# tongdaxu/VQ-VAE-from-Gaussian-VAE

Hardware: AMD Instinct MI355X
Metric: images/sec encode+quantize+decode, 256x256, codebook 2^16 (higher is better)
Workload: dtype f32

## Files before the change

vq-vae-from-gaussian-vae_amd/csrc/gq_unet_aux.h:

```cpp
#pragma once
#include "gq_common.h"
#include "gq_stats.h"

namespace gqhip {

typedef unsigned u32x4_t __attribute__((ext_vector_type(4)));

__device__ __forceinline__ float silu_f32(float x) {
  const float d = 1.0f + __expf(-x);
  const float r = __builtin_amdgcn_rcpf(d);
  const float q = x * r;
  const float q1 = __builtin_fmaf(__builtin_fmaf(-d, q, x), r, q);
  return d > 1e37f ? q : q1;
}

template <int SILU, typename VEC>
__device__ __forceinline__ VEC gn_act(VEC v, VEC a, VEC sh) {
  v = v * a + sh;
  if (SILU) {
#pragma unroll
    for (int e = 0; e < (int)(sizeof(VEC) / sizeof(float)); ++e) v[e] = silu_f32(v[e]);
  }
  return v;
}
__global__ __launch_bounds__(256) void gn_stats_nhwc_kernel(const float *__restrict__ x,
                                                            const float *__restrict__ pre_bias,
                                                            int64_t *__restrict__ stats, int C, long HW, int cpg,
                                                            int slabs) {
  __shared__ int64_t red[kStatWords * 64];
  const int groups = C / cpg, quads = C / 4, lanes = 256 / quads;
  const long b = blockIdx.x / slabs;
  const int slab = blockIdx.x % slabs;
  const long per = (HW + slabs - 1) / slabs;
  const long lo = slab * per, hi = lo + per < HW ? lo + per : HW;
  const int q = threadIdx.x % quads, pl = threadIdx.x / quads;
// ... 246 lines not shown
          d[i][j] = reinterpret_cast<const f32x4 *>(x)[((wt.b * H + sy) * W + sx) * C4 + wt.q];
      }
    f32x4 w[4][4];
#pragma unroll
    for (int j = 0; j < 4; ++j) {
      w[0][j] = d[0][j] - d[2][j];
      w[1][j] = d[1][j] + d[2][j];
      w[2][j] = d[2][j] - d[1][j];
      w[3][j] = d[1][j] - d[3][j];
    }
    f32x4 *v = reinterpret_cast<f32x4 *>(V);
#pragma unroll
    for (int i = 0; i < 4; ++i) {
      v[((long)(4 * i + 0) * tiles + wt.tile) * C4 + wt.q] = w[i][0] - w[i][2];
      v[((long)(4 * i + 1) * tiles + wt.tile) * C4 + wt.q] = w[i][1] + w[i][2];
      v[((long)(4 * i + 2) * tiles + wt.tile) * C4 + wt.q] = w[i][2] - w[i][1];
      v[((long)(4 * i + 3) * tiles + wt.tile) * C4 + wt.q] = w[i][1] - w[i][3];
    }
  }
}
template <int F16X3>
__global__ __launch_bounds__(256) void wino_in_nhwc_kernel(const float *__restrict__ x, void *__restrict__ V, int H, int W,
                                                           int C4, long tiles, long total, float scale) {
  if constexpr (F16X3 == 0) wino_in_items_f32(x, static_cast<float *>(V), H, W, C4, tiles, total);
  else wino_in_items<F16X3, uint32_t>(x, V, H, W, C4, tiles, total, scale);
}
template <int F16X3>
__global__ __launch_bounds__(256) void wino_in_nhwc_wide_kernel(const float *__restrict__ x, void *__restrict__ V, int H, int W,
                                                                int C4, long tiles, long total, float scale) {
  if constexpr (F16X3 == 0) wino_in_items_f32(x, static_cast<float *>(V), H, W, C4, tiles, total);
  else wino_in_items<F16X3, uint64_t>(x, V, H, W, C4, tiles, total, scale);
}

template <int SILU, int F16X3, typename OFF>
__device__ __forceinline__ void wino_in_gn_items(const float *__restrict__ x, const float *__restrict__ gamma,
                                                 const float *__restrict__ beta, const float *__restrict__ pre_bias,
                                                 const int64_t *__restrict__ stats, void *__restrict__ V, int H, int W, int C4,
                                                 int cpg, double eps, long tiles, long total, float scale) {
  typedef WinoVRow<F16X3, f32x4> VR;
  const int groups = 4 * C4 / cpg;
  const OFF px = (OFF)C4 * sizeof(f32x4), row = (OFF)W * px;
  const OFF part = (OFF)C4 * VR::VB;
  const uint64_t plane = (uint64_t)tiles * VR::PARTS * part;
  const char *xb = reinterpret_cast<const char *>(x);
  for (OFF t = (OFF)blockIdx.x * 256 + threadIdx.x; t < (OFF)total; t += (OFF)gridDim.x * 256) {
    const WinoTile<OFF> wt = wino_tile<2>(t, C4, H, W);
    char *vk = wino_plane0(static_cast<char *>(V));
    const int g = (4 * wt.q) / cpg;
    const GnGroup gg = gn_group(stats + kStatWords * ((long)wt.b * groups + g), (double)cpg * (double)H * (double)W, eps);
    f32x4 a, sh;
#pragma unroll
    for (int k = 0; k < 4; ++k) {
      const GnAffine f = gn_channel(gg, gamma, beta, pre_bias, 4 * wt.q + k);
      a[k] = f.a;
      sh[k] = f.sh;
    }
    const OFF xq = wt.b * ((OFF)H * row) + (OFF)wt.q * sizeof(f32x4);
    OFF ro[4], co[4];
    float rin[4], cin[4];
    wino_taps<4>(2 * wt.th - 1, H, row, xq, ro, rin);
    wino_taps<4>(2 * wt.tw - 1, W, px, (OFF)0, co, cin);
    f32x4 d[4][4];
#pragma unroll
    for (int i = 0; i < 4; ++i)
#pragma unroll
      for (int j = 0; j < 4; ++j) {
        d[i][j] = *reinterpret_cast<const f32x4 *>(xb + (OFF)(ro[i] + co[j]));
      }
#pragma unroll
    for (int i = 0; i < 4; ++i)
#pragma unroll
      for (int j = 0; j < 4; ++j) {
        const float inb = rin[i] * cin[j];
        d[i][j] = gn_act<SILU>(d[i][j], a, sh) * inb;
      }
    f32x4 w[4][4];
#pragma unroll
    for (int j = 0; j < 4; ++j) {
      w[0][j] = d[0][j] - d[2][j];
      w[1][j] = d[1][j] + d[2][j];
      w[2][j] = d[2][j] - d[1][j];
      w[3][j] = d[1][j] - d[3][j];
    }
    const OFF at = wt.tile * (VR::PARTS * part) + (OFF)wt.q * VR::VB;
#pragma unroll
    for (int i = 0; i < 4; ++i) {
      wino_store_v<F16X3>(vk, at, part, w[i][0] - w[i][2], scale);
      vk += plane;
      wino_store_v<F16X3>(vk, at, part, w[i][1] + w[i][2], scale);
      vk += plane;
      wino_store_v<F16X3>(vk, at, part, w[i][2] - w[i][1], scale);
      vk += plane;
      wino_store_v<F16X3>(vk, at, part, w[i][1] - w[i][3], scale);
      vk += plane;
    }
  }
}
#define GQ_WINO_GN_ARGS                                                                                                        \
  const float *__restrict__ x, const float *__restrict__ gamma, const float *__restrict__ beta,                               \
      const float *__restrict__ pre_bias, const int64_t *__restrict__ stats, void *__restrict__ V, int H, int W, int CV, int cpg, \
      double eps, long tiles, long total, float scale
template <int SILU, int F16X3>
__global__ __launch_bounds__(256) __attribute__((amdgpu_waves_per_eu(3, 4))) void wino_in_gn_nhwc_kernel(GQ_WINO_GN_ARGS) {
  wino_in_gn_items<SILU, F16X3, uint32_t>(x, gamma, beta, pre_bias, stats, V, H, W, CV, cpg, eps, tiles, total, scale);
}
template <int SILU, int F16X3>
__global__ __launch_bounds__(256) void wino_in_gn_nhwc_wide_kernel(GQ_WINO_GN_ARGS) {
  wino_in_gn_items<SILU, F16X3, uint64_t>(x, gamma, beta, pre_bias, stats, V, H, W, CV, cpg, eps, tiles, total, scale);
}

template <int F16X3, typename OFF>
__device__ __forceinline__ void wino4_in_items(const float *__restrict__ x, void *__restrict__ V, int H, int W, int C4, long tiles,
                                               long total, float scale) {
  typedef WinoVRow<F16X3, f32x4> VR;
  const OFF px = (OFF)C4 * sizeof(f32x4), row = (OFF)W * px;
  const OFF part = (OFF)C4 * VR::VB;
  const uint64_t plane = (uint64_t)tiles * VR::PARTS * part;
  const char *xb = reinterpret_cast<const char *>(x);
  for (OFF t = (OFF)blockIdx.x * 256 + threadIdx.x; t < (OFF)total; t += (OFF)gridDim.x * 256) {
    const WinoTile<OFF> wt = wino_tile<4>(t, C4, H, W);
    char *vk = wino_plane0(static_cast<char *>(V));
    const OFF xq = wt.b * ((OFF)H * row) + (OFF)wt.q * sizeof(f32x4);
    OFF ro[6], co[6];
    bool rin[6], cin[6];
    wino_taps<6>(4 * wt.th - 1, H, row, xq, ro, rin);
    wino_taps<6>(4 * wt.tw - 1, W, px, (OFF)0, co, cin);
    f32x4 w[6][6];
#pragma unroll
    for (int j = 0; j < 6; ++j) {
      f32x4 col[6], o[6];
#pragma unroll
      for (int i = 0; i < 6; ++i) {
        col[i] = f32x4{0.f, 0.f, 0.f, 0.f};
        if (rin[i] && cin[j]) col[i] = *reinterpret_cast<const f32x4 *>(xb + (OFF)(ro[i] + co[j]));
      }
      wino4_bt(col, o);
#pragma unroll
      for (int i = 0; i < 6; ++i) w[i][j] = o[i];
    }
    const OFF at = wt.tile * (VR::PARTS * part) + (OFF)wt.q * VR::VB;
#pragma unroll
    for (int i = 0; i < 6; ++i) {
// ... 582 lines not shown
```

vq-vae-from-gaussian-vae_amd/csrc/gq_wino_range.h:

```cpp
#pragma once
#include <stdint.h>

#include <initializer_list>

namespace gqhip {

inline bool wino_product_le(uint64_t a, uint64_t b, uint64_t limit) { return a == 0 || b <= limit / a; }

inline bool wino_offsets_fit_u32(int64_t B, int64_t H, int64_t W, int64_t C, int64_t tile, int64_t plane_bytes_per_channel) {
  if (B < 0 || H < 1 || W < 1 || C < 1 || tile < 1 || plane_bytes_per_channel < 1) return false;
  const uint64_t limit = 1ull << 32;
  uint64_t tensor = 4, plane = (uint64_t)plane_bytes_per_channel;
  for (uint64_t f : {(uint64_t)B, (uint64_t)H, (uint64_t)W, (uint64_t)C}) {
    if (!wino_product_le(tensor, f, limit)) return false;
    tensor *= f;
  }
  for (uint64_t f : {(uint64_t)B, (uint64_t)(H / tile), (uint64_t)(W / tile), (uint64_t)C}) {
    if (!wino_product_le(plane, f, limit)) return false;
    plane *= f;
  }
  return true;
}

}
```

vq-vae-from-gaussian-vae_amd/csrc/gqhip_unet.hip:

```cpp
#include "gqhip.h"

#include <hip/hip_ext.h>
#include <hip/hip_runtime.h>

#include <cstdlib>
#include <initializer_list>
#include <cstring>

#include "gqhip_internal.h"
#include "gq_unet_aux.h"
#include "gq_wino_range.h"
#include "gq_wino_gemm.h"
#include "gq_conv3.h"
#include "gq_conv_f32.h"
#include "gq_attn.h"
#include "gq_attn_bwd.h"

using namespace gqhip;

namespace {
thread_local int g_stats_prezeroed = 0;
inline hipError_t stats_zero(void *p, size_t bytes, hipStream_t st) {
  return g_stats_prezeroed ? hipSuccess : hipMemsetAsync(p, 0, bytes, st);
}

constexpr int kGo = -1;

dim3 grid1d(long total, long cap) {
  const long blocks = (total + 255) / 256;
  return dim3((unsigned)(blocks > cap ? cap : blocks));
}

int nhwc_slabs(int64_t C, int64_t HW) {
  const int lanes = (int)(256 / (C / 4));
  int slabs = (int)((HW + (int64_t)lanes * 16 - 1) / ((int64_t)lanes * 16));
  if (slabs > 1024) slabs = 1024;
  return slabs < 1 ? 1 : slabs;
}

int gn_check(int64_t B, int64_t C, int64_t HW, int64_t groups, bool ptrs_ok, bool nhwc) {
  if (B < 0 || C < 1 || HW < 1 || groups < 1 || C % groups != 0) return GQHIP_ERR_INVALID_ARG;
  if (B == 0) return GQHIP_OK;
  if (!ptrs_ok) return GQHIP_ERR_INVALID_ARG;
  if (nhwc && ((C / groups) % 4 != 0 || 256 % (C / 4) != 0 || groups > 64)) return GQHIP_ERR_INVALID_ARG;
  return kGo;
}

bool wino_shape_ok(int64_t B, int64_t H, int64_t W, int64_t C, int64_t tile) {
  return (tile == 2 || tile == 4) && B >= 0 && H >= tile && W >= tile && H % tile == 0 && W % tile == 0 && C >= 4 && C % 4 == 0;
}
bool wino_u32(int64_t B, int64_t H, int64_t W, int64_t C, int64_t tile, int64_t plane_bytes_per_channel) {
  const char *knob = getenv("GQHIP_WINO_WIDE");
  return !(knob && !strcmp(knob, "1")) && wino_offsets_fit_u32(B, H, W, C, tile, plane_bytes_per_channel);
}

bool one_of(int64_t v, std::initializer_list<int64_t> values) {
  for (int64_t w : values)
    if (v == w) return true;
  return false;
}
}

extern "C" {

int gqhip_stats_prezeroed(int on) {
  g_stats_prezeroed = on != 0;
  return GQHIP_OK;
}

int gn_silu_f32(const float *x, const float *gamma, const float *beta, const float *pre_bias_or_null, float *y,
                int64_t B, int64_t C, int64_t HW, int64_t groups, double eps, int apply_silu, int layout,
                int64_t *stats_ws, void *stream) {
  const bool nhwc = layout == GQHIP_LAYOUT_NHWC;
  if (int rc = gn_check(B, C, HW, groups, x && gamma && beta && y && stats_ws, nhwc); rc != kGo) return rc;
  hipStream_t st = static_cast<hipStream_t>(stream);
  const int64_t bg = B * groups, cpg = C / groups, chunk = cpg * HW;
  if (nhwc) {
    if (stats_zero(stats_ws, sizeof(int64_t) * kStatWords * bg, st) != hipSuccess) return check_launch();
    const int slabs = nhwc_slabs(C, HW);
    hipLaunchKernelGGL(gn_stats_nhwc_kernel, dim3((unsigned)(B * slabs)), dim3(256), 0, st, x, pre_bias_or_null,
                       stats_ws, (int)C, (long)HW, (int)cpg, slabs);
    int rc = check_launch();
    if (rc != GQHIP_OK) return rc;
    return launch(apply_silu ? gn_apply_nhwc_kernel<1> : gn_apply_nhwc_kernel<0>, dim3((unsigned)(B * slabs)), dim3(256), 0, st, x,
                  gamma, beta, y, stats_ws, pre_bias_or_null, (int)C, (long)HW, (int)cpg, eps, slabs);
  }
// ... 111 lines not shown
  wp.nnb = (int)(Cout / cols);
  wp.mtiles = tiles / rows; wp.ntile_total = P * wp.mtiles; wp.tiles_per_xcd = (wp.ntile_total + 7) / 8;
  const long blocks = 8 * wp.tiles_per_xcd * wp.nnb;
  if (blocks > 0x7fffffffL) return GQHIP_ERR_INVALID_ARG;
  hipStream_t st = static_cast<hipStream_t>(stream);
  switch (tiling) {
    case WinoGemmTiling::k128x256: hipLaunchKernelGGL(wino_gemm_f16x2_k64_kernel<1>, dim3((unsigned)blocks), dim3(256), 0, st, wp); break;
    case WinoGemmTiling::k256x256: hipLaunchKernelGGL(wino_gemm_f16x2_k64_kernel<2>, dim3((unsigned)blocks), dim3(512), 0, st, wp); break;
    case WinoGemmTiling::k256x128: hipLaunchKernelGGL(wino_gemm_f16x2_kernel, dim3((unsigned)blocks), dim3(256), 0, st, wp); break;
  }
  return check_launch();
}

int gn_stats_f32(const float *x, const float *pre_bias_or_null, int64_t B, int64_t C, int64_t HW, int64_t groups,
                 int64_t *stats_out, void *stream) {
  if (int rc = gn_check(B, C, HW, groups, x && stats_out, true); rc != kGo) return rc;
  const int64_t cpg = C / groups;
  hipStream_t st = static_cast<hipStream_t>(stream);
  if (stats_zero(stats_out, sizeof(int64_t) * kStatWords * B * groups, st) != hipSuccess) return check_launch();
  const int slabs = nhwc_slabs(C, HW);
  return launch(gn_stats_nhwc_kernel, dim3((unsigned)(B * slabs)), dim3(256), 0, st, x, pre_bias_or_null, stats_out,
                (int)C, (long)HW, (int)cpg, slabs);
}

static int wino_in_gn_impl(int tile, int f16, const float *x, const float *gamma, const float *beta,
                           const float *pre_bias_or_null, const int64_t *stats, void *V, int64_t B, int64_t H, int64_t W,
                           int64_t C, int64_t groups, double eps, int apply_silu, float scale, void *stream) {
  if (!wino_shape_ok(B, H, W, C, tile) || groups < 1 || C % groups != 0 || (C / groups) % 4 != 0 || !(scale > 0.f))
    return GQHIP_ERR_INVALID_ARG;
  if (B == 0) return GQHIP_OK;
  if (!x || !gamma || !beta || !stats || !V) return GQHIP_ERR_INVALID_ARG;
  const int vw = (tile == 4 && f16 != 0) ? 2 : 4;
  const long tiles = (long)(B * (H / tile) * (W / tile)), total = tiles * (C / vw);
  const dim3 grid = grid1d(total, 32768);
  hipStream_t st = static_cast<hipStream_t>(stream);
  const bool u32 = wino_u32(B, H, W, C, tile, f16 == 1 ? 6 : 4);
#define GQ_WGN(K, ...)                                                                                                       \
  hipLaunchKernelGGL((u32 ? K##_kernel<__VA_ARGS__> : K##_wide_kernel<__VA_ARGS__>), grid, dim3(256), 0, st, x, gamma, beta, \
                     pre_bias_or_null, stats, V, (int)H, (int)W, (int)(C / vw), (int)(C / groups), eps, tiles, total, scale)
  if (tile == 4) {
    if (apply_silu) {
      if (f16 == 2) GQ_WGN(wino4_in_gn_nhwc, 1, 2, 2); else if (f16 == 1) GQ_WGN(wino4_in_gn_nhwc, 1, 1, 2);
      else GQ_WGN(wino4_in_gn_nhwc, 1, 0, 4);
    } else {
      if (f16 == 2) GQ_WGN(wino4_in_gn_nhwc, 0, 2, 2); else if (f16 == 1) GQ_WGN(wino4_in_gn_nhwc, 0, 1, 2);
      else GQ_WGN(wino4_in_gn_nhwc, 0, 0, 4);
    }
  } else {
    if (apply_silu) {
      if (f16 == 2) GQ_WGN(wino_in_gn_nhwc, 1, 2); else if (f16 == 1) GQ_WGN(wino_in_gn_nhwc, 1, 1);
      else GQ_WGN(wino_in_gn_nhwc, 1, 0);
    } else {
      if (f16 == 2) GQ_WGN(wino_in_gn_nhwc, 0, 2); else if (f16 == 1) GQ_WGN(wino_in_gn_nhwc, 0, 1);
      else GQ_WGN(wino_in_gn_nhwc, 0, 0);
    }
  }
#undef GQ_WGN
  return check_launch();
}

int wino_in_gn_nhwc_f32(const float *x, const float *gamma, const float *beta, const float *pre_bias_or_null,
                        const int64_t *stats, float *V, int64_t B, int64_t H, int64_t W, int64_t C, int64_t groups,
                        double eps, int apply_silu, void *stream) {
  return wino_in_gn_impl(2, 0, x, gamma, beta, pre_bias_or_null, stats, V, B, H, W, C, groups, eps, apply_silu, 1.0f, stream);
}

int wino4_in_gn_nhwc_f32(const float *x, const float *gamma, const float *beta, const float *pre_bias_or_null,
                         const int64_t *stats, float *V, int64_t B, int64_t H, int64_t W, int64_t C, int64_t groups,
                         double eps, int apply_silu, void *stream) {
// ... 457 lines not shown
```

vq-vae-from-gaussian-vae_amd/csrc/gq_conv3.h:

```cpp
#pragma once
#include <type_traits>

#include "gq_common.h"
#include "gq_epilogue.h"
#include "gq_stats.h"
#include "gq_wino_gemm.h"

namespace gqhip {

constexpr int kC3TH = 8, kC3TW = 32;
constexpr int kC3PH = kC3TH + 2, kC3PW = kC3TW + 2;
constexpr int kC3Pix = kC3PH * kC3PW;
constexpr int kC3RS = 48;
constexpr int kC3Plane = kC3PH * kC3RS * 32;
constexpr int kC3Buf = 2 * kC3Plane;
constexpr int kC3Pieces = kC3Pix * 4;
constexpr int kC3Loads = (kC3Pieces + 255) / 256;

__device__ __forceinline__ int conv3_lds_off(int R, int x, int half) {
  return (R * kC3RS + x) * 32 + 16 * (half ^ ((x >> 3) & 1));
}

struct Conv3Params {
  const _Float16 *Xs;
// ... 75 lines not shown
    double *mine = part + (wn * 64 + lane) * 4;
    if (wm == 0) {
      if (p.res) epi_store<3, true>(acc, stage, lane, p.y, p.res, o, slice, 4 * cout, p.mscale, pb, st);
      else epi_store<2, true>(acc, stage, lane, p.y, nullptr, o, slice, 4 * cout, p.mscale, pb, st);
      mine[0] = st.v0; mine[1] = st.s; mine[2] = st.ss; mine[3] = (double)st.n;
    }
    __syncthreads();
    if (wm == 1) {
      st.v0 = mine[0]; st.s = mine[1]; st.ss = mine[2]; st.n = (int)mine[3];
      if (p.res) epi_store<3, true>(acc, stage, lane, p.y, p.res, o, slice, 4 * cout, p.mscale, pb, st);
      else epi_store<2, true>(acc, stage, lane, p.y, nullptr, o, slice, 4 * cout, p.mscale, pb, st);
      stat_partial_flush(red + kStatWords * (n / p.cpg), st);
    }
  }
  __syncthreads();
  const int gpb = 128 / p.cpg, groups = cout / p.cpg;
  if (tid < kStatWords * gpb) stat_flush_word(p.stats + kStatWords * (t.b * groups + t.nb * gpb) + tid, red[tid]);
}

#define GQ_C3_ZERO_ACC(acc)                                                                                         \
  _Pragma("unroll") for (int rr = 0; rr < 4; ++rr) _Pragma("unroll") for (int j = 0; j < 2; ++j) acc[rr][j] =       \
      f32x16{0.f, 0.f, 0.f, 0.f, 0.f, 0.f, 0.f, 0.f, 0.f, 0.f, 0.f, 0.f, 0.f, 0.f, 0.f, 0.f}

struct Conv3GnParams {
  Conv3Params c;
  const float *x;
  const float *gamma, *beta, *pre_bias;
  const int64_t *stats_in;
  int cin, cpg_in;
  double eps;
  float scale;
};

#ifdef GQHIP_CLOCK_STAMPS
__device__ unsigned long long g_c3_stamps[4 * 8192];
#endif
template <int SILU, int COUT>
__global__ __launch_bounds__(256, 2) void conv3x3_gn_f16x3_kernel(const Conv3GnParams pp) {
  typedef _Float16 f16x4 __attribute__((ext_vector_type(4)));
  const Conv3Params &p = pp.c;
  __shared__ __attribute__((aligned(16))) unsigned char sA[2 * kC3Buf];
  __shared__ int64_t red[kStatWords * 32];
  __shared__ __attribute__((aligned(16))) float sAff[2][512];
  const int tid = threadIdx.x, lane = tid & 63, wave = __builtin_amdgcn_readfirstlane(tid >> 6);
  const int c = lane & 31, h = lane >> 5, wm = wave >> 1, wn = wave & 1;
#ifdef GQHIP_CLOCK_STAMPS
  const unsigned long long st_r0 = __builtin_amdgcn_s_memrealtime();
#endif
  Conv3Tile t;
  if (!conv3_tile(p, t)) return;
  const int H = p.H, W = p.W, cin = pp.cin;
  red[tid] = 0;
  {
    const int groups = cin / pp.cpg_in;
    const double n = (double)pp.cpg_in * (double)H * (double)W;
    for (int ch = tid; ch < cin; ch += 256) {
      const GnAffine f = gn_channel(gn_group(pp.stats_in + kStatWords * (t.b * groups + ch / pp.cpg_in), n, pp.eps), pp.gamma, pp.beta, pp.pre_bias, ch);
      sAff[0][ch] = f.a;
      sAff[1][ch] = f.sh;
    }
  }
  const int w = tid & 3, qs = tid >> 2;
  int goff[kC3Loads];
  unsigned inb = 0;
#pragma unroll
  for (int i = 0; i < kC3Loads; ++i) {
    int q = qs + 64 * i;
    q = q < kC3Pix ? q : kC3Pix - 1;
    const int R = q / kC3PW, px = q % kC3PW;
    const int gy = t.y0 - 1 + R, gx = t.x0 - 1 + px;
    const bool in = gy >= 0 && gy < H && gx >= 0 && gx < W;
    const int cy = clamp_index(gy, H), cx = clamp_index(gx, W);
    goff[i] = (cy * W + cx) * cin + 4 * w;
    inb |= (unsigned)(in ? 1 : 0) << i;
  }
  const float *xb = pp.x + t.b * (long)H * W * cin;
  f32x4 st[3];
  auto issue = [&](int i, int chunk) { st[i % 3] = *reinterpret_cast<const f32x4 *>(xb + goff[i] + chunk * 16); };
  auto convert = [&](int i, int chunk, int buf) {
    const int q = qs + 64 * i;
    if (q >= kC3Pix) return;
    const f32x4 a4 = *reinterpret_cast<const f32x4 *>(&sAff[0][chunk * 16 + 4 * w]);
    const f32x4 sh4 = *reinterpret_cast<const f32x4 *>(&sAff[1][chunk * 16 + 4 * w]);
    const f32x4 v = gn_act<SILU>(st[i % 3], a4, sh4) * (((inb >> i) & 1) ? pp.scale : 0.f);
    f16x4 hi, lo;
#pragma unroll
    for (int e = 0; e < 4; ++e) {
      hi[e] = (_Float16)v[e];
      lo[e] = (_Float16)(v[e] - (float)hi[e]);
    }
    const int off = buf * kC3Buf + conv3_lds_off(q / kC3PW, q % kC3PW, w >> 1) + 8 * (w & 1);
    *reinterpret_cast<f16x4 *>(&sA[off]) = hi;
    *reinterpret_cast<f16x4 *>(&sA[off + kC3Plane]) = lo;
  };

  f32x16 acc[4][2];
  GQ_C3_ZERO_ACC(acc);
  int aoff[3];
#pragma unroll
  for (int dx = 0; dx < 3; ++dx) aoff[dx] = conv3_lds_off(4 * wm, c + dx, h);
  const unsigned char *wbase = reinterpret_cast<const unsigned char *>(p.Wf) + (4 * t.nb + 2 * wn) * 128 * 16;
  const int wl = lane * 16;
  const long wstep = (long)p.nnb * (512 * 16);
  f16x8 bs[3][4];
  auto load_b = [&](int ks, f16x8 (&dst)[4]) {
    const unsigned char *s = wbase + ks * wstep;
#pragma unroll
    for (int k = 0; k < 4; ++k) dst[k] = *reinterpret_cast<const f16x8 *>(s + k * 1024 + wl);
  };
  const int nks = p.nch * 9;
  load_b(0, bs[0]);
  load_b(1, bs[1]);
  __syncthreads();
  for (int i0 = 0; i0 < kC3Loads; i0 += 3) {
#pragma unroll
    for (int i = 0; i < 3; ++i) issue(i0 + i, 0);
#pragma unroll
    for (int i = 0; i < 3; ++i) convert(i0 + i, 0, 0);
  }
  __syncthreads();

#ifdef GQHIP_CLOCK_STAMPS
  const unsigned long long st_r1 = __builtin_amdgcn_s_memrealtime();
#endif
  for (int chunk = 0; chunk < p.nch; ++chunk) {
    const bool more = chunk + 1 < p.nch;
    const unsigned char *A = sA + (chunk & 1) * kC3Buf;
    const int nbuf = (chunk + 1) & 1;
#pragma unroll
    for (int tap = 0; tap < 9; ++tap) {
      const int ks = chunk * 9 + tap;
#if !(defined(GQHIP_ABL) && (GQHIP_ABL & 128))
      load_b(ks + 2 < nks ? ks + 2 : nks - 1, bs[(tap + 2) % 3]);
#endif
      conv3_tap(A + aoff[tap % 3], tap / 3, bs[tap % 3], acc);
#if !(defined(GQHIP_ABL) && (GQHIP_ABL & 64))
      if (more) {
        if (tap >= 3) convert(tap - 3, chunk + 1, nbuf);
        if (tap < kC3Loads) issue(tap, chunk + 1);
      }
#endif
      __builtin_amdgcn_sched_barrier(0);
    }
    __syncthreads();
  }
#ifdef GQHIP_CLOCK_STAMPS
  const unsigned long long st_r2 = __builtin_amdgcn_s_memrealtime();
#endif
#if defined(GQHIP_ABL) && (GQHIP_ABL & 512)
  if (acc[0][0][0] == 12345.678f)
#endif
  conv3_epilogue<COUT>(p, t, acc, sA, red, wave, wm, wn);
#ifdef GQHIP_CLOCK_STAMPS
  if (tid == 0 && blockIdx.x < 8192) {
    unsigned long long *o = g_c3_stamps + 4 * blockIdx.x;
    o[0] = st_r0;
    o[1] = __builtin_amdgcn_s_memrealtime();
    o[2] = ((st_r1 - st_r0) << 32) | (st_r2 - st_r0);
    o[3] = ((unsigned long long)__builtin_amdgcn_s_getreg((31 << 11) | 20) << 32) | (unsigned)__builtin_amdgcn_s_getreg((31 << 11) | 4);
  }
#endif
}



struct Conv1Params {
  Conv3Params c;
  const float *x;
  const float *pre_bias;
  const float *scales_dev;
  float scale;
  int cin;
  const float *gamma, *beta;
  const int64_t *stats_in;
  int cpg_in;
  double eps;
  _Float16 *Q3, *K3, *V3;
  float sq, sv;
// ... 67 lines not shown
#pragma unroll
    for (int j = 0; j < 2; ++j) acc[rr][j] = f32x16{0.f, 0.f, 0.f, 0.f, 0.f, 0.f, 0.f, 0.f, 0.f, 0.f, 0.f, 0.f, 0.f, 0.f, 0.f, 0.f};
  const int aoff = (RR * wm) * 1024 + c * 32 + 16 * (h ^ ((c >> 3) & 1));
  const unsigned char *wbase = reinterpret_cast<const unsigned char *>(p.Wf) + (4 * t.nb + 2 * wn) * 128 * 16;
  const int wl = lane * 16;
  const long wstep = (long)p.nnb * (512 * 16);
  f16x8 b0[4], b1[4];
  auto load_b = [&](int ks, f16x8 (&dst)[4]) {
    const unsigned char *s = wbase + ks * wstep;
#pragma unroll
    for (int k = 0; k < 4; ++k) dst[k] = *reinterpret_cast<const f16x8 *>(s + k * 1024 + wl);
  };
  auto kstep = [&](const unsigned char *A, const f16x8 (&bq)[4]) {
#pragma unroll
    for (int rr = 0; rr < RR; ++rr) {
      const f16x8 ah = *reinterpret_cast<const f16x8 *>(A + aoff + rr * 1024);
      const f16x8 al = *reinterpret_cast<const f16x8 *>(A + aoff + rr * 1024 + kPlane);
#pragma unroll
      for (int j = 0; j < 2; ++j) {
        acc[rr][j] = __builtin_amdgcn_mfma_f32_32x32x16_f16(ah, bq[2 * j], acc[rr][j], 0, 0, 0);
        acc[rr][j] = __builtin_amdgcn_mfma_f32_32x32x16_f16(ah, bq[2 * j + 1], acc[rr][j], 0, 0, 0);
        acc[rr][j] = __builtin_amdgcn_mfma_f32_32x32x16_f16(al, bq[2 * j], acc[rr][j], 0, 0, 0);
      }
    }
  };
  const int nks = 2 * nst;
  load_b(0, b0);
  issue(0);
  if constexpr (GN != 0) __syncthreads();
  affine(0);
#pragma unroll
  for (int i = 0; i < NI; ++i) convert(i, 0);
  __syncthreads();
  for (int s = 0; s < nst; ++s) {
    const bool more = s + 1 < nst;
    const unsigned char *A = sA + (s & 1) * kStage;
    const int nbuf = (s + 1) & 1;
    load_b(2 * s + 1, b1);
    if (more) issue(s + 1);
    kstep(A, b0);
    __builtin_amdgcn_sched_barrier(0);
    load_b(2 * s + 2 < nks ? 2 * s + 2 : nks - 1, b0);
    kstep(A + kChunk, b1);
    if (more) {
      affine(s + 1);
#pragma unroll
      for (int i = 0; i < NI; ++i) convert(i, nbuf);
    }
    __builtin_amdgcn_sched_barrier(0);
    __syncthreads();
  }
  if constexpr (SPLIT != 0) {
    const int C = p.cout / 3, col = t.nb * 128, third = col / C;
    const int n = wn * 64 + 4 * (lane & 15), cc = col - third * C + n;
    const long L = (long)p.H * 32, tok = (long)(t.y0 + RR * wm) * 32 + (lane >> 4);
    f32x4 pb = {0.f, 0.f, 0.f, 0.f};
    if (p.bias) {
#pragma unroll
      for (int e = 0; e < 4; ++e) pb[e] = p.bias[col + n + e];
    }
    float *stage = reinterpret_cast<float *>(sA + wave * kEpiWaveBytes);
    if (third < 2) {
      _Float16 *dst = third == 0 ? pp.Q3 : pp.K3;
      epi_store_split(acc, stage, lane, dst, (t.b * L + tok) * 3 * C + cc, 32L * 3 * C, 4L * 3 * C, (long)C, third == 0, p.mscale,
                      pb, pp.sq);
    } else {
      epi_store_split(acc, stage, lane, pp.V3, (t.b * 3 * L + tok) * C + cc, 32L * C, 4L * C, L * C, false, p.mscale, pb, pp.sv);
    }
  } else {
    conv3_epilogue<COUT>(p, t, acc, sA, red, wave, wm, wn);
  }
}

struct Conv3S2Params {
  Conv3Params c;
  const float *x;
  const float *scales_dev;
  float scale;
  int cin, Hin, Win;
};

template <int COUT>
__global__ __launch_bounds__(256, 2) void conv3x3s2_f16x3_kernel(const Conv3S2Params pp) {
// ... 111 lines not shown
  float scale;
  int cin;
};

template <int COUT>
__global__ __launch_bounds__(256, 2) void upconv2x_f16x3_kernel(const Upconv2Params pp) {
  typedef _Float16 f16x4 __attribute__((ext_vector_type(4)));
  Conv3Params p = pp.c;
  __shared__ __attribute__((aligned(16))) unsigned char sA[2 * kC3Buf];
  __shared__ int64_t red[kStatWords * 32];
  const int tid = threadIdx.x, lane = tid & 63, wave = __builtin_amdgcn_readfirstlane(tid >> 6);
  const int c = lane & 31, h = lane >> 5, wm = wave >> 1, wn = wave & 1;
  Conv3Tile t;
  if (!conv3_tile(p, t)) return;
  const int pa = (int)blockIdx.y >> 1, pb = (int)blockIdx.y & 1;
  red[tid] = 0;
  const float scale = pp.scales_dev ? pp.scales_dev[0] : pp.scale;
  if (pp.scales_dev) p.mscale = pp.scales_dev[1];
  const int cin = pp.cin, nch = p.nch, H = p.H, W = p.W;
  constexpr int PR = kC3TH + 1, PC = kC3TW + 1, NP = 5;
  const int w = tid & 3, qs = tid >> 2;
  const float *xb = pp.x + t.b * (long)H * W * cin + 4 * w;
  int goff[NP], loff[NP];
  unsigned inb = 0;
#pragma unroll
  for (int i = 0; i < NP; ++i) {
    const int q = qs + 64 * i;
    const int qq = q < PR * PC ? q : PR * PC - 1;
    const int R = qq / PC, X = qq % PC;
    const int gy = t.y0 + R + pa - 1, gx = t.x0 + X + pb - 1;
    const bool in = gy >= 0 && gy < H && gx >= 0 && gx < W;
    const int cy = gy < 0 ? 0 : (gy >= H ? H - 1 : gy), cx = gx < 0 ? 0 : (gx >= W ? W - 1 : gx);
    goff[i] = (cy * W + cx) * cin;
    loff[i] = q < PR * PC ? conv3_lds_off(R, X, w >> 1) + 8 * (w & 1) : -1;
    inb |= (unsigned)(in ? 1 : 0) << i;
  }
  f32x4 st[NP];
  auto issue = [&](int chunk) {
#pragma unroll
    for (int i = 0; i < NP; ++i) st[i] = *reinterpret_cast<const f32x4 *>(xb + goff[i] + chunk * 16);
  };
  auto commit = [&](int buf) {
#pragma unroll
    for (int i = 0; i < NP; ++i) {
      if (loff[i] < 0) continue;
      const f32x4 v = st[i] * (((inb >> i) & 1) ? scale : 0.f);
      f16x4 hi, lo;
#pragma unroll
      for (int e = 0; e < 4; ++e) {
        hi[e] = (_Float16)v[e];
        lo[e] = (_Float16)(v[e] - (float)hi[e]);
      }
      unsigned char *d = sA + buf * kC3Buf + loff[i];
      *reinterpret_cast<f16x4 *>(d) = hi;
      *reinterpret_cast<f16x4 *>(d + kC3Plane) = lo;
    }
  };
  f32x16 acc[4][2];
  GQ_C3_ZERO_ACC(acc);
  int aoff[2];
#pragma unroll
  for (int dx = 0; dx < 2; ++dx) aoff[dx] = conv3_lds_off(4 * wm, c + dx, h);
  const long wstep = (long)p.nnb * (512 * 16);
  const int nks = 4 * nch;
  const unsigned char *wbase = reinterpret_cast<const unsigned char *>(p.Wf) + (long)blockIdx.y * nks * wstep +
                               (4 * t.nb + 2 * wn) * 128 * 16;
  const int wl = lane * 16;
  f16x8 b0[4], b1[4], b2[4];
  auto load_b = [&](int ks, f16x8 (&dst)[4]) {
    const unsigned char *s = wbase + (long)(ks < nks ? ks : nks - 1) * wstep;
#pragma unroll
    for (int k = 0; k < 4; ++k) dst[k] = *reinterpret_cast<const f16x8 *>(s + k * 1024 + wl);
  };
  load_b(0, b0);
  load_b(1, b1);
  issue(0);
  commit(0);
  __syncthreads();
  int ks = 0;
  for (int chunk = 0; chunk < nch; ++chunk) {
    const bool more = chunk + 1 < nch;
    if (more) issue(chunk + 1);
    const unsigned char *A = sA + (chunk & 1) * kC3Buf;
#pragma unroll
    for (int ti = 0; ti < 4; ++ti) {
      load_b(ks + 2, b2);
      conv3_tap(A + aoff[ti & 1], ti >> 1, b0, acc);
#pragma unroll
      for (int k = 0; k < 4; ++k) {
        b0[k] = b1[k];
        b1[k] = b2[k];
      }
      ++ks;
      __builtin_amdgcn_sched_barrier(0);
    }
    if (more) commit((chunk + 1) & 1);
    __syncthreads();
  }
  constexpr int cout = COUT;
  const int n = wn * 64 + 4 * (lane & 15);
  f32x4 bias4 = {0.f, 0.f, 0.f, 0.f};
  if (p.bias) {
#pragma unroll
    for (int e = 0; e < 4; ++e) bias4[e] = p.bias[t.nb * 128 + n + e];
  }
  float *stage = reinterpret_cast<float *>(sA + wave * kEpiWaveBytes);
  const long W2 = 2L * W;
  const long o = ((t.b * 2L * H + 2 * (t.y0 + 4 * wm) + pa) * W2 + 2 * (t.x0 + (lane >> 4)) + pb) * cout + t.nb * 128 + n;
  StatPartial sp;
  if (!p.stats) {
    epi_store<1, false>(acc, stage, lane, p.y, nullptr, o, 2 * W2 * cout, 8 * cout, p.mscale, bias4, sp);
    return;
  }
  epi_store<1, true>(acc, stage, lane, p.y, nullptr, o, 2 * W2 * cout, 8 * cout, p.mscale, bias4, sp);
  stat_partial_flush(red + kStatWords * (n / p.cpg), sp);
  __syncthreads();
  const int gpb = 128 / p.cpg, groups = cout / p.cpg;
  if (tid < kStatWords * gpb) stat_flush_word(p.stats + kStatWords * (t.b * groups + t.nb * gpb) + tid, red[tid]);
}

template <int SILU, int COUT>
__global__ __launch_bounds__(256) void conv3x3_gn_small_kernel(const float *__restrict__ x, const float *__restrict__ gamma,
                                                               const float *__restrict__ beta,
                                                               const float *__restrict__ pre_bias,
                                                               const int64_t *__restrict__ stats, const float *__restrict__ w,
                                                               const float *__restrict__ bias, float *__restrict__ y, int H,
                                                               int W, int C, int cpg, double eps) {
  constexpr int PW = 18, PS = 36;
  __shared__ __attribute__((aligned(16))) float sX[PW * PW * PS];
  __shared__ __attribute__((aligned(16))) float sAff[2][512];
  const int tid = threadIdx.x, tx = tid & 15, ty = tid >> 4;
// ... 56 lines not shown
```

Before: 521.4.

## Add strip-tiled Winograd input transform with block-shared GroupNorm affine

Adds a strip kernel for the F(2x2) Winograd input transform fused with GroupNorm and SiLU, used for f16 variants when C<=512. Each block handles a contiguous strip of tiles from one image and precomputes that image's per-channel GN scale and shift once into shared memory. This replaces the per-thread recomputation from int64 stats. Block indices are swizzled across 8 XCD groups so neighbouring strips share L2, and sched_barriers are inserted to keep loads grouped ahead of math and stores. The cost is a __syncthreads per block, plus possible load imbalance when a strip is short.

Result: no change. 520.2 (-0.2%).

```diff
diff --git a/vq-vae-from-gaussian-vae_amd/csrc/gq_unet_aux.h b/vq-vae-from-gaussian-vae_amd/csrc/gq_unet_aux.h
--- a/vq-vae-from-gaussian-vae_amd/csrc/gq_unet_aux.h
+++ b/vq-vae-from-gaussian-vae_amd/csrc/gq_unet_aux.h
@@ -1,6 +1,7 @@
 #pragma once
 #include "gq_common.h"
 #include "gq_stats.h"
+#include "gq_wino_range.h"
 
 namespace gqhip {
 
@@ -313,6 +314,60 @@
   else wino_in_items<F16X3, uint64_t>(x, V, H, W, C4, tiles, total, scale);
 }
 
+__device__ __forceinline__ void gn_fold_image(float (&aff)[2][kWinoFoldC], const int64_t *__restrict__ stats,
+                                              const float *__restrict__ gamma, const float *__restrict__ beta,
+                                              const float *__restrict__ pre_bias, int64_t b, int C, int cpg, double n, double eps) {
+  const int groups = C / cpg;
+  for (int ch = threadIdx.x; ch < C; ch += kWinoBlock) {
+    const GnAffine f = gn_channel(gn_group(stats + kStatWords * (b * groups + ch / cpg), n, eps), gamma, beta, pre_bias, ch);
+    aff[0][ch] = f.a;
+    aff[1][ch] = f.sh;
+  }
+}
+
+template <int SILU, int F16X3, typename OFF>
+__device__ __forceinline__ void wino_in_gn_item(const char *xb, OFF xq, int th, int tw, int H, int W, OFF row, OFF px, f32x4 a,
+                                                f32x4 sh, char *vk, uint64_t plane, OFF at, OFF part, float scale) {
+  OFF ro[4], co[4];
+  float rin[4], cin[4];
+  wino_taps<4>(2 * th - 1, H, row, xq, ro, rin);
+  wino_taps<4>(2 * tw - 1, W, px, (OFF)0, co, cin);
+  f32x4 d[4][4];
+#pragma unroll
+  for (int i = 0; i < 4; ++i)
+#pragma unroll
+    for (int j = 0; j < 4; ++j) {
+      d[i][j] = *reinterpret_cast<const f32x4 *>(xb + (OFF)(ro[i] + co[j]));
+    }
+  __builtin_amdgcn_sched_barrier(0);
+#pragma unroll
+  for (int i = 0; i < 4; ++i)
+#pragma unroll
+    for (int j = 0; j < 4; ++j) {
+      const float inb = rin[i] * cin[j];
+      d[i][j] = gn_act<SILU>(d[i][j], a, sh) * inb;
+    }
+  f32x4 w[4][4];
+#pragma unroll
+  for (int j = 0; j < 4; ++j) {
+    w[0][j] = d[0][j] - d[2][j];
+    w[1][j] = d[1][j] + d[2][j];
+    w[2][j] = d[2][j] - d[1][j];
+    w[3][j] = d[1][j] - d[3][j];
+  }
+#pragma unroll
+  for (int i = 0; i < 4; ++i) {
+    wino_store_v<F16X3>(vk, at, part, w[i][0] - w[i][2], scale);
+    vk += plane;
+    wino_store_v<F16X3>(vk, at, part, w[i][1] + w[i][2], scale);
+    vk += plane;
+    wino_store_v<F16X3>(vk, at, part, w[i][2] - w[i][1], scale);
+    vk += plane;
+    wino_store_v<F16X3>(vk, at, part, w[i][1] - w[i][3], scale);
+    vk += plane;
+    __builtin_amdgcn_sched_barrier(0);
+  }
+}
 template <int SILU, int F16X3, typename OFF>
 __device__ __forceinline__ void wino_in_gn_items(const float *__restrict__ x, const float *__restrict__ gamma,
                                                  const float *__restrict__ beta, const float *__restrict__ pre_bias,
@@ -337,44 +392,32 @@
       sh[k] = f.sh;
     }
     const OFF xq = wt.b * ((OFF)H * row) + (OFF)wt.q * sizeof(f32x4);
-    OFF ro[4], co[4];
-    float rin[4], cin[4];
-    wino_taps<4>(2 * wt.th - 1, H, row, xq, ro, rin);
-    wino_taps<4>(2 * wt.tw - 1, W, px, (OFF)0, co, cin);
-    f32x4 d[4][4];
-#pragma unroll
-    for (int i = 0; i < 4; ++i)
-#pragma unroll
-      for (int j = 0; j < 4; ++j) {
-        d[i][j] = *reinterpret_cast<const f32x4 *>(xb + (OFF)(ro[i] + co[j]));
-      }
-#pragma unroll
-    for (int i = 0; i < 4; ++i)
-#pragma unroll
-      for (int j = 0; j < 4; ++j) {
-        const float inb = rin[i] * cin[j];
-        d[i][j] = gn_act<SILU>(d[i][j], a, sh) * inb;
-      }
-    f32x4 w[4][4];
-#pragma unroll
-    for (int j = 0; j < 4; ++j) {
-      w[0][j] = d[0][j] - d[2][j];
-      w[1][j] = d[1][j] + d[2][j];
-      w[2][j] = d[2][j] - d[1][j];
-      w[3][j] = d[1][j] - d[3][j];
-    }
     const OFF at = wt.tile * (VR::PARTS * part) + (OFF)wt.q * VR::VB;
-#pragma unroll
-    for (int i = 0; i < 4; ++i) {
-      wino_store_v<F16X3>(vk, at, part, w[i][0] - w[i][2], scale);
-      vk += plane;
-      wino_store_v<F16X3>(vk, at, part, w[i][1] + w[i][2], scale);
-      vk += plane;
-      wino_store_v<F16X3>(vk, at, part, w[i][2] - w[i][1], scale);
-      vk += plane;
-      wino_store_v<F16X3>(vk, at, part, w[i][1] - w[i][3], scale);
-      vk += plane;
-    }
+    wino_in_gn_item<SILU, F16X3, OFF>(xb, xq, wt.th, wt.tw, H, W, row, px, a, sh, vk, plane, at, part, scale);
+  }
+}
+template <int SILU, int F16X3, typename OFF>
+__device__ __forceinline__ void wino_in_gn_strip_items(const float *__restrict__ x, const float *__restrict__ gamma,
+                                                       const float *__restrict__ beta, const float *__restrict__ pre_bias,
+                                                       const int64_t *__restrict__ stats, void *__restrict__ V, int H, int W, int C4,
+                                                       int cpg, double eps, long tiles, const WinoStrips &strips, float scale) {
+  typedef WinoVRow<F16X3, f32x4> VR;
+  __shared__ __attribute__((aligned(16))) float sAff[2][kWinoFoldC];
+  const WinoStrip strip = wino_strip(strips, blockIdx.x);
+  if (strip.tiles == 0) return;
+  gn_fold_image(sAff, stats, gamma, beta, pre_bias, strip.image, 4 * C4, cpg, (double)cpg * (double)H * (double)W, eps);
+  const OFF px = (OFF)C4 * sizeof(f32x4), row = (OFF)W * px;
+  const OFF part = (OFF)C4 * VR::VB;
+  const uint64_t plane = (uint64_t)tiles * VR::PARTS * part;
+  const char *xb = reinterpret_cast<const char *>(x) + (uint64_t)strip.image * ((uint64_t)H * row);
+  char *vs = static_cast<char *>(V) + (uint64_t)(strip.image * strips.tpi + strip.first) * (VR::PARTS * part);
+  const WinoStep step = wino_step(C4, strips.TW);
+  __syncthreads();
+  for (WinoWalk w = wino_walk_first(step, strip, threadIdx.x); w.tl < strip.tiles; wino_walk_next(step, w)) {
+    char *vk = wino_plane0(vs);
+    const f32x4 a = *reinterpret_cast<const f32x4 *>(&sAff[0][4 * w.q]), sh = *reinterpret_cast<const f32x4 *>(&sAff[1][4 * w.q]);
+    const OFF at = (OFF)w.tl * (VR::PARTS * part) + (OFF)w.q * VR::VB;
+    wino_in_gn_item<SILU, F16X3, OFF>(xb, (OFF)w.q * sizeof(f32x4), w.th, w.tw, H, W, row, px, a, sh, vk, plane, at, part, scale);
   }
 }
 #define GQ_WINO_GN_ARGS                                                                                                        \
@@ -389,6 +432,19 @@
 __global__ __launch_bounds__(256) void wino_in_gn_nhwc_wide_kernel(GQ_WINO_GN_ARGS) {
   wino_in_gn_items<SILU, F16X3, uint64_t>(x, gamma, beta, pre_bias, stats, V, H, W, CV, cpg, eps, tiles, total, scale);
 }
+#define GQ_WINO_GN_STRIP_ARGS                                                                                                  \
+  const float *__restrict__ x, const float *__restrict__ gamma, const float *__restrict__ beta,                               \
+      const float *__restrict__ pre_bias, const int64_t *__restrict__ stats, void *__restrict__ V, int H, int W, int CV, int cpg, \
+      double eps, long tiles, WinoStrips strips, float scale
+template <int SILU, int F16X3>
+__global__ __launch_bounds__(256) __attribute__((amdgpu_waves_per_eu(3, 4))) void wino_in_gn_strip_kernel(GQ_WINO_GN_STRIP_ARGS) {
+  wino_in_gn_strip_items<SILU, F16X3, uint32_t>(x, gamma, beta, pre_bias, stats, V, H, W, CV, cpg, eps, tiles, strips, scale);
+}
+template <int SILU, int F16X3>
+__global__ __launch_bounds__(256) void wino_in_gn_strip_wide_kernel(GQ_WINO_GN_STRIP_ARGS) {
+  wino_in_gn_strip_items<SILU, F16X3, uint64_t>(x, gamma, beta, pre_bias, stats, V, H, W, CV, cpg, eps, tiles, strips, scale);
+}
+#undef GQ_WINO_GN_STRIP_ARGS
 
 template <int F16X3, typename OFF>
 __device__ __forceinline__ void wino4_in_items(const float *__restrict__ x, void *__restrict__ V, int H, int W, int C4, long tiles,
diff --git a/vq-vae-from-gaussian-vae_amd/csrc/gq_wino_range.h b/vq-vae-from-gaussian-vae_amd/csrc/gq_wino_range.h
--- a/vq-vae-from-gaussian-vae_amd/csrc/gq_wino_range.h
+++ b/vq-vae-from-gaussian-vae_amd/csrc/gq_wino_range.h
@@ -22,4 +22,88 @@
   return true;
 }
 
+#if defined(__HIPCC__)
+#define GQ_WINO_HD __host__ __device__ __forceinline__
+#else
+#define GQ_WINO_HD inline
+#endif
+
+constexpr int kWinoBlock = 256;
+constexpr int kWinoFoldC = 512;
+
+struct WinoStrips {
+  int64_t tpi;
+  int64_t per_image;
+  int64_t count;
+  int64_t per_xcd;
+  int64_t group;
+  int TW, len;
+};
+GQ_WINO_HD WinoStrips wino_strips(int64_t B, int64_t TH, int64_t TW, int len, int64_t group) {
+  WinoStrips s;
+  s.tpi = TH * TW;
+  s.per_image = (s.tpi + len - 1) / len;
+  s.count = B * s.per_image;
+  s.group = group;
+  s.per_xcd = (s.count + 8 * group - 1) / (8 * group) * group;
+  s.TW = (int)TW;
+  s.len = len;
+  return s;
 }
+struct WinoStrip {
+  int64_t image, first;
+  int th, tw, tiles;
+};
+GQ_WINO_HD int64_t wino_strip_index(const WinoStrips &s, int64_t vb) {
+  const int64_t k = vb >> 3, chunk = k / s.group;
+  return (chunk * 8 + (vb & 7)) * s.group + (k - chunk * s.group);
+}
+GQ_WINO_HD WinoStrip wino_strip(const WinoStrips &s, int64_t vb) {
+  WinoStrip r = {0, 0, 0, 0, 0};
+  const int64_t strip = wino_strip_index(s, vb);
+  if (strip >= s.count) return r;
+  r.image = strip / s.per_image;
+  r.first = (strip - r.image * s.per_image) * s.len;
+  r.th = (int)(r.first / s.TW);
+  r.tw = (int)(r.first - (int64_t)r.th * s.TW);
+  r.tiles = (int)(s.tpi - r.first < s.len ? s.tpi - r.first : s.len);
+  return r;
+}
+struct WinoStep {
+  int CV, TW, dq, dth, dtw;
+  int dtl;
+};
+struct WinoWalk {
+  int q, tl, th, tw;
+};
+GQ_WINO_HD WinoStep wino_step(int CV, int TW) {
+  WinoStep s;
+  s.CV = CV;
+  s.TW = TW;
+  s.dq = kWinoBlock % CV;
+  s.dtl = kWinoBlock / CV;
+  s.dth = s.dtl / TW;
+  s.dtw = s.dtl % TW;
+  return s;
+}
+GQ_WINO_HD WinoWalk wino_walk_first(const WinoStep &s, const WinoStrip &strip, int t) {
+  WinoWalk w;
+  w.q = t % s.CV;
+  w.tl = t / s.CV;
+  const int c = strip.tw + w.tl;
+  w.th = strip.th + c / s.TW;
+  w.tw = c % s.TW;
+  return w;
+}
+GQ_WINO_HD void wino_walk_next(const WinoStep &s, WinoWalk &w) {
+  w.q += s.dq;
+  const int cq = w.q >= s.CV;
+  w.q -= cq ? s.CV : 0;
+  w.tl += s.dtl + cq;
+  w.tw += s.dtw + cq;
+  const int ct = w.tw >= s.TW;
+  w.tw -= ct ? s.TW : 0;
+  w.th += s.dth + ct;
+}
+
+}
diff --git a/vq-vae-from-gaussian-vae_amd/csrc/gqhip_unet.hip b/vq-vae-from-gaussian-vae_amd/csrc/gqhip_unet.hip
--- a/vq-vae-from-gaussian-vae_amd/csrc/gqhip_unet.hip
+++ b/vq-vae-from-gaussian-vae_amd/csrc/gqhip_unet.hip
@@ -52,6 +52,14 @@
 bool wino_u32(int64_t B, int64_t H, int64_t W, int64_t C, int64_t tile, int64_t plane_bytes_per_channel) {
   const char *knob = getenv("GQHIP_WINO_WIDE");
   return !(knob && !strcmp(knob, "1")) && wino_offsets_fit_u32(B, H, W, C, tile, plane_bytes_per_channel);
+}
+
+int wino_strip_len(int64_t CV) {
+  if (const char *knob = getenv("GQHIP_WINO_STRIP")) {
+    const long v = strtol(knob, nullptr, 10);
+    return v < 0 ? 0 : v > 4096 ? 4096 : (int)v;
+  }
+  return (int)((kWinoBlock + CV - 1) / CV);
 }
 
 bool one_of(int64_t v, std::initializer_list<int64_t> values) {
@@ -229,9 +237,22 @@
   if (!x || !gamma || !beta || !stats || !V) return GQHIP_ERR_INVALID_ARG;
   const int vw = (tile == 4 && f16 != 0) ? 2 : 4;
   const long tiles = (long)(B * (H / tile) * (W / tile)), total = tiles * (C / vw);
+  hipStream_t st = static_cast<hipStream_t>(stream);
+  const bool u32 = wino_u32(B, H, W, C, tile, f16 == 1 ? 6 : 4);
+  const int strip_len = (tile == 2 && f16 != 0 && C <= kWinoFoldC) ? wino_strip_len(C / vw) : 0;
+  const WinoStrips strips = wino_strips(B, H / tile, W / tile, strip_len > 0 ? strip_len : 1, (W / tile + strip_len - 1) / (strip_len > 0 ? strip_len : 1));
+  if (strip_len > 0 && 8 * strips.per_xcd <= 0x7fffffffL) {
+    const dim3 grid((unsigned)(8 * strips.per_xcd));
+#define GQ_WGN(...)                                                                                                                \
+  hipLaunchKernelGGL((u32 ? wino_in_gn_strip_kernel<__VA_ARGS__> : wino_in_gn_strip_wide_kernel<__VA_ARGS__>), grid, dim3(kWinoBlock), \
+                     0, st, x, gamma, beta, pre_bias_or_null, stats, V, (int)H, (int)W, (int)(C / vw), (int)(C / groups), eps, tiles, \
+                     strips, scale)
+    if (apply_silu) { if (f16 == 2) GQ_WGN(1, 2); else GQ_WGN(1, 1); }
+    else { if (f16 == 2) GQ_WGN(0, 2); else GQ_WGN(0, 1); }
+#undef GQ_WGN
+    return check_launch();
+  }
   const dim3 grid = grid1d(total, 32768);
-  hipStream_t st = static_cast<hipStream_t>(stream);
-  const bool u32 = wino_u32(B, H, W, C, tile, f16 == 1 ? 6 : 4);
 #define GQ_WGN(K, ...)                                                                                                       \
   hipLaunchKernelGGL((u32 ? K##_kernel<__VA_ARGS__> : K##_wide_kernel<__VA_ARGS__>), grid, dim3(256), 0, st, x, gamma, beta, \
                      pre_bias_or_null, stats, V, (int)H, (int)W, (int)(C / vw), (int)(C / groups), eps, tiles, total, scale)
```

## Interleave conversion VALU work with MFMAs via sched_group_barrier in conv kernels

Applied to the files above, without the earlier changes.

Peels the last chunk/stage into a compile-time 'no more' specialization so the prefetch/convert branches become constexpr. Adds sched_group_barrier patterns that alternate one MFMA with several VALU ops, so the fp32→f16 hi/lo conversion of the next chunk hides under matrix work. Applies this to the conv3x3+GN kernel, the RR==2 Winograd GEMM path, and the upsample conv, where the commit is split per piece and spread across taps. Out-of-range pieces are clamped and their redundant writes land on a duplicate pixel rather than being branched around, trading a little extra work for branch-free code. There is a risk of register pressure or forced schedules that stall.

Result: faster. 517.7 before, 530.9 after, median of 6 (+2.5%).

```diff
diff --git a/vq-vae-from-gaussian-vae_amd/csrc/gq_conv3.h b/vq-vae-from-gaussian-vae_amd/csrc/gq_conv3.h
--- a/vq-vae-from-gaussian-vae_amd/csrc/gq_conv3.h
+++ b/vq-vae-from-gaussian-vae_amd/csrc/gq_conv3.h
@@ -131,6 +131,9 @@
   float scale;
 };
 
+#ifndef GQHIP_C3_VALU_PER_MFMA
+#define GQHIP_C3_VALU_PER_MFMA 3
+#endif
 #ifdef GQHIP_CLOCK_STAMPS
 __device__ unsigned long long g_c3_stamps[4 * 8192];
 #endif
@@ -177,8 +180,7 @@
   f32x4 st[3];
   auto issue = [&](int i, int chunk) { st[i % 3] = *reinterpret_cast<const f32x4 *>(xb + goff[i] + chunk * 16); };
   auto convert = [&](int i, int chunk, int buf) {
-    const int q = qs + 64 * i;
-    if (q >= kC3Pix) return;
+    const int q = qs + 64 * i < kC3Pix ? qs + 64 * i : kC3Pix - 1;
     const f32x4 a4 = *reinterpret_cast<const f32x4 *>(&sAff[0][chunk * 16 + 4 * w]);
     const f32x4 sh4 = *reinterpret_cast<const f32x4 *>(&sAff[1][chunk * 16 + 4 * w]);
     const f32x4 v = gn_act<SILU>(st[i % 3], a4, sh4) * (((inb >> i) & 1) ? pp.scale : 0.f);
@@ -222,8 +224,8 @@
 #ifdef GQHIP_CLOCK_STAMPS
   const unsigned long long st_r1 = __builtin_amdgcn_s_memrealtime();
 #endif
-  for (int chunk = 0; chunk < p.nch; ++chunk) {
-    const bool more = chunk + 1 < p.nch;
+  auto run_chunk = [&](int chunk, auto more_tag) {
+    constexpr bool more = decltype(more_tag)::value;
     const unsigned char *A = sA + (chunk & 1) * kC3Buf;
     const int nbuf = (chunk + 1) & 1;
 #pragma unroll
@@ -234,15 +236,26 @@
 #endif
       conv3_tap(A + aoff[tap % 3], tap / 3, bs[tap % 3], acc);
 #if !(defined(GQHIP_ABL) && (GQHIP_ABL & 64))
-      if (more) {
+      if constexpr (more) {
         if (tap >= 3) convert(tap - 3, chunk + 1, nbuf);
         if (tap < kC3Loads) issue(tap, chunk + 1);
+#if GQHIP_C3_VALU_PER_MFMA > 0
+        if (tap >= 3) {
+#pragma unroll
+          for (int m = 0; m < 24; ++m) {
+            __builtin_amdgcn_sched_group_barrier(0x008, 1, 0);
+            __builtin_amdgcn_sched_group_barrier(0x002, GQHIP_C3_VALU_PER_MFMA, 0);
+          }
+        }
+#endif
       }
 #endif
       __builtin_amdgcn_sched_barrier(0);
     }
     __syncthreads();
-  }
+  };
+  for (int chunk = 0; chunk + 1 < p.nch; ++chunk) run_chunk(chunk, std::true_type{});
+  run_chunk(p.nch - 1, std::false_type{});
 #ifdef GQHIP_CLOCK_STAMPS
   const unsigned long long st_r2 = __builtin_amdgcn_s_memrealtime();
 #endif
@@ -376,23 +389,51 @@
 #pragma unroll
   for (int i = 0; i < NI; ++i) convert(i, 0);
   __syncthreads();
-  for (int s = 0; s < nst; ++s) {
-    const bool more = s + 1 < nst;
-    const unsigned char *A = sA + (s & 1) * kStage;
-    const int nbuf = (s + 1) & 1;
-    load_b(2 * s + 1, b1);
-    if (more) issue(s + 1);
-    kstep(A, b0);
-    __builtin_amdgcn_sched_barrier(0);
-    load_b(2 * s + 2 < nks ? 2 * s + 2 : nks - 1, b0);
-    kstep(A + kChunk, b1);
-    if (more) {
-      affine(s + 1);
-#pragma unroll
-      for (int i = 0; i < NI; ++i) convert(i, nbuf);
-    }
-    __builtin_amdgcn_sched_barrier(0);
-    __syncthreads();
+  if constexpr (RR == 2) {
+    auto run_stage = [&](int s, auto more_tag) {
+      constexpr bool more = decltype(more_tag)::value;
+      const unsigned char *A = sA + (s & 1) * kStage;
+      const int nbuf = (s + 1) & 1;
+      load_b(2 * s + 1, b1);
+      if constexpr (more) issue(s + 1);
+      kstep(A, b0);
+      __builtin_amdgcn_sched_barrier(0);
+      if constexpr (more) affine(s + 1);
+      load_b(2 * s + 2 < nks ? 2 * s + 2 : nks - 1, b0);
+      kstep(A + kChunk, b1);
+      if constexpr (more) {
+#pragma unroll
+        for (int i = 0; i < NI; ++i) convert(i, nbuf);
+#pragma unroll
+        for (int m = 0; m < 6 * RR; ++m) {
+          __builtin_amdgcn_sched_group_barrier(0x008, 1, 0);
+          __builtin_amdgcn_sched_group_barrier(0x002, 8, 0);
+        }
+      }
+      __builtin_amdgcn_sched_barrier(0);
+      __syncthreads();
+    };
+    for (int s = 0; s + 1 < nst; ++s) run_stage(s, std::true_type{});
+    run_stage(nst - 1, std::false_type{});
+  } else {
+    for (int s = 0; s < nst; ++s) {
+      const bool more = s + 1 < nst;
+      const unsigned char *A = sA + (s & 1) * kStage;
+      const int nbuf = (s + 1) & 1;
+      load_b(2 * s + 1, b1);
+      if (more) issue(s + 1);
+      kstep(A, b0);
+      __builtin_amdgcn_sched_barrier(0);
+      load_b(2 * s + 2 < nks ? 2 * s + 2 : nks - 1, b0);
+      kstep(A + kChunk, b1);
+      if (more) {
+        affine(s + 1);
+#pragma unroll
+        for (int i = 0; i < NI; ++i) convert(i, nbuf);
+      }
+      __builtin_amdgcn_sched_barrier(0);
+      __syncthreads();
+    }
   }
   if constexpr (SPLIT != 0) {
     const int C = p.cout / 3, col = t.nb * 128, third = col / C;
@@ -570,7 +611,7 @@
     const bool in = gy >= 0 && gy < H && gx >= 0 && gx < W;
     const int cy = gy < 0 ? 0 : (gy >= H ? H - 1 : gy), cx = gx < 0 ? 0 : (gx >= W ? W - 1 : gx);
     goff[i] = (cy * W + cx) * cin;
-    loff[i] = q < PR * PC ? conv3_lds_off(R, X, w >> 1) + 8 * (w & 1) : -1;
+    loff[i] = conv3_lds_off(R, X, w >> 1) + 8 * (w & 1);
     inb |= (unsigned)(in ? 1 : 0) << i;
   }
   f32x4 st[NP];
@@ -578,21 +619,17 @@
 #pragma unroll
     for (int i = 0; i < NP; ++i) st[i] = *reinterpret_cast<const f32x4 *>(xb + goff[i] + chunk * 16);
   };
-  auto commit = [&](int buf) {
-#pragma unroll
-    for (int i = 0; i < NP; ++i) {
-      if (loff[i] < 0) continue;
-      const f32x4 v = st[i] * (((inb >> i) & 1) ? scale : 0.f);
-      f16x4 hi, lo;
-#pragma unroll
-      for (int e = 0; e < 4; ++e) {
-        hi[e] = (_Float16)v[e];
-        lo[e] = (_Float16)(v[e] - (float)hi[e]);
-      }
-      unsigned char *d = sA + buf * kC3Buf + loff[i];
-      *reinterpret_cast<f16x4 *>(d) = hi;
-      *reinterpret_cast<f16x4 *>(d + kC3Plane) = lo;
-    }
+  auto commit_piece = [&](int i, int buf) {
+    const f32x4 v = st[i] * (((inb >> i) & 1) ? scale : 0.f);
+    f16x4 hi, lo;
+#pragma unroll
+    for (int e = 0; e < 4; ++e) {
+      hi[e] = (_Float16)v[e];
+      lo[e] = (_Float16)(v[e] - (float)hi[e]);
+    }
+    unsigned char *d = sA + buf * kC3Buf + loff[i];
+    *reinterpret_cast<f16x4 *>(d) = hi;
+    *reinterpret_cast<f16x4 *>(d + kC3Plane) = lo;
   };
   f32x16 acc[4][2];
   GQ_C3_ZERO_ACC(acc);
@@ -613,13 +650,15 @@
   load_b(0, b0);
   load_b(1, b1);
   issue(0);
-  commit(0);
+#pragma unroll
+  for (int i = 0; i < NP; ++i) commit_piece(i, 0);
   __syncthreads();
   int ks = 0;
-  for (int chunk = 0; chunk < nch; ++chunk) {
-    const bool more = chunk + 1 < nch;
-    if (more) issue(chunk + 1);
+  auto run_chunk = [&](int chunk, auto more_tag) {
+    constexpr bool more = decltype(more_tag)::value;
+    if constexpr (more) issue(chunk + 1);
     const unsigned char *A = sA + (chunk & 1) * kC3Buf;
+    const int nbuf = (chunk + 1) & 1;
 #pragma unroll
     for (int ti = 0; ti < 4; ++ti) {
       load_b(ks + 2, b2);
@@ -630,11 +669,30 @@
         b1[k] = b2[k];
       }
       ++ks;
+      if constexpr (more) {
+        if (ti == 2) {
+          commit_piece(0, nbuf);
+          commit_piece(1, nbuf);
+        }
+        if (ti == 3) {
+          commit_piece(2, nbuf);
+          commit_piece(3, nbuf);
+          commit_piece(4, nbuf);
+        }
+        if (ti >= 2) {
+#pragma unroll
+          for (int m = 0; m < 24; ++m) {
+            __builtin_amdgcn_sched_group_barrier(0x008, 1, 0);
+            __builtin_amdgcn_sched_group_barrier(0x002, 3, 0);
+          }
+        }
+      }
       __builtin_amdgcn_sched_barrier(0);
     }
-    if (more) commit((chunk + 1) & 1);
     __syncthreads();
-  }
+  };
+  for (int chunk = 0; chunk + 1 < nch; ++chunk) run_chunk(chunk, std::true_type{});
+  run_chunk(nch - 1, std::false_type{});
   constexpr int cout = COUT;
   const int n = wn * 64 + 4 * (lane & 15);
   f32x4 bias4 = {0.f, 0.f, 0.f, 0.f};
```
